# yukara-ikemiya/friendly-stable-audio-tools

Hardware: AMD Instinct MI355X
Metric: audio-seconds/sec @44.1kHz stereo, 100-step DPM++, SA-Open-1.0 shape (higher is better)
Workload: dtype fp16; 1 GPU; Stable-Audio-Open-1.0 DiT shape (24 layers, D=1536, S=1025, CFG 7 -> 2 sequences/prompt) + Oobleck decode, 1 prompt(s)/GPU x 47.55 s, 100 DPM-Solver++(3M) SDE steps; prompts_per_gpu=1, codec_dtype=fp16, sampler_steps=100, layernorm=fused, cross_attention=fused, sample_size=2097152, parallelism=dp1 (rank-strided prompts, one all-gather)

## Files before the change

### friendly-stable-audio-tools_amd/csrc/gemm_bf16.hip

```cpp
#include <stdlib.h>

#include <type_traits>

#include "attn_core.h"
#include <algorithm>

#include "sat_common.h"

namespace {

template <int EPI, int MI, int NI, bool LNC = false, bool QKN = false>
__device__ __forceinline__ void gemm_epilogue(const GemmArgs& g, f32x16 (&acc)[MI][NI], const int mw, const int nw, const int half,
                                              const int l31, const float2* ln = nullptr, const float* lc1 = nullptr,
                                              const float* lc2 = nullptr) {
    const int M = g.M, N = g.N;
    (void)N;

    if constexpr (EPI == EPI_F32) {
        float* __restrict__ C = g.C;
        const int ldc = g.ldc;
        float bia[NI];
#pragma unroll
        for (int j = 0; j < NI; ++j) bia[j] = g.bias ? g.bias[nw + j * 32 + l31] : 0.f;
        const bool accum = g.accumulate != 0;
// ... 344 lines not shown
            const int m = mw + i * 32 + l31;
            const int mc = m < M ? m : M - 1;
            const int b = mc / S;
            const int s = mc - b * S;
            const int ob = (kind & 4) ? ((b * S) & 3) : 0;
            if constexpr (LNC) {
                const float2 st = ln[i * 32 + l31];
#pragma unroll
                for (int j = 0; j < 2; ++j)
#pragma unroll
                    for (int q = 0; q < 4; ++q) {
                        const f32x4 c1 = *reinterpret_cast<const f32x4*>(lc1 + j * 32 + q * 8 + 4 * half);
                        const f32x4 c2 = *reinterpret_cast<const f32x4*>(lc2 + j * 32 + q * 8 + 4 * half);
#pragma unroll
                        for (int e = 0; e < 4; ++e) acc[i][j][4 * q + e] = st.y * (acc[i][j][4 * q + e] - st.x * c1[e]) + c2[e];
                    }
            }
            if constexpr (QKN) {
                if (kind & 16) {
                    float ss = 0.f;
#pragma unroll
                    for (int j = 0; j < 2; ++j)
#pragma unroll
                        for (int r = 0; r < 16; ++r) ss += acc[i][j][r] * acc[i][j][r];
                    unsigned a = __float_as_uint(ss), b = a;
                    half_swap(a, b);
                    const float inv = rsqrtf(fmaxf(__uint_as_float(a) + __uint_as_float(b), 1e-24f));
#pragma unroll
                    for (int j = 0; j < 2; ++j)
#pragma unroll
                        for (int r = 0; r < 16; ++r) acc[i][j][r] *= inv;
                }
            }
            if (kind & 2) {
                if constexpr (!ROPE_PRE) {
                    rcs[i][0] = *reinterpret_cast<const f32x4*>(he.rope_cos + (size_t)s * 16 + 4 * half);
                    rcs[i][1] = *reinterpret_cast<const f32x4*>(he.rope_cos + (size_t)s * 16 + 8 + 4 * half);
                    rsn[i][0] = *reinterpret_cast<const f32x4*>(he.rope_sin + (size_t)s * 16 + 4 * half);
                    rsn[i][1] = *reinterpret_cast<const f32x4*>(he.rope_sin + (size_t)s * 16 + 8 + 4 * half);
                }
                const f32x4 cs0 = rcs[i][0], cs1 = rcs[i][1], sn0 = rsn[i][0], sn1 = rsn[i][1];
#pragma unroll
                for (int r = 0; r < 8; ++r) {
                    const float cs = (r < 4) ? cs0[r & 3] : cs1[r & 3];
                    const float sn = (r < 4) ? sn0[r & 3] : sn1[r & 3];
                    const float x1 = acc[i][0][r], x2 = acc[i][0][r + 8];
                    acc[i][0][r] = x1 * cs - x2 * sn;
                    acc[i][0][r + 8] = x2 * cs + x1 * sn;
                }
            }
            if (kind & 8) {
#pragma unroll
                for (int j = 0; j < 2; ++j)
#pragma unroll
                    for (int r = 0; r < 16; ++r) acc[i][j][r] *= he.qscale;
            }
            op_t* row = dst + ((size_t)(b * he.heads + head) * Spad + s + ob) * 64 + 8 * half;
#pragma unroll
            for (int j = 0; j < 2; ++j) {
                unsigned pk[8];
#pragma unroll
                for (int q = 0; q < 4; ++q) {
                    pk[2 * q] = pack_op2(acc[i][j][4 * q], acc[i][j][4 * q + 1]);
                    pk[2 * q + 1] = pack_op2(acc[i][j][4 * q + 2], acc[i][j][4 * q + 3]);
                }
                half_swap(pk[0], pk[2]);
                half_swap(pk[1], pk[3]);
                half_swap(pk[4], pk[6]);
                half_swap(pk[5], pk[7]);
                if (qfrag) {
#pragma unroll
                    for (int e = 0; e < 8; ++e) qfrag[j][e] = pk[e];
                    continue;
                }
                if (m < M) {
                    *reinterpret_cast<u32x4*>(row + j * 32) = u32x4{pk[0], pk[1], pk[2], pk[3]};
                    *reinterpret_cast<u32x4*>(row + j * 32 + 16) = u32x4{pk[4], pk[5], pk[6], pk[7]};
                }
            }
        }
    }
}

template <int MI>
__device__ __forceinline__ void stage_rows32(float* ep, const f32x16 (&acc)[MI][2], const int i, const int lane) {
    const int half = lane >> 5, l31 = lane & 31;
#pragma unroll
    for (int j = 0; j < 2; ++j)
#pragma unroll
        for (int r = 0; r < 16; ++r) ep[((r & 3) + 8 * (r >> 2) + 4 * half) * 64 + j * 32 + l31] = acc[i][j][r];
}
template <int MB>
__device__ __forceinline__ void stage_rows32(float* ep, const f32x4 (&acc)[MB][4], const int i, const int lane) {
    const int l15 = lane & 15, q = lane >> 4;
#pragma unroll
    for (int rb = 0; rb < 2; ++rb)
#pragma unroll
        for (int cb = 0; cb < 4; ++cb)
#pragma unroll
            for (int r = 0; r < 4; ++r) ep[(rb * 16 + 4 * q + r) * 64 + cb * 16 + l15] = acc[2 * i + rb][cb][r];
}

template <int MI, bool PRE = false, typename Acc>
__device__ __forceinline__ void gemm_epilogue_f32_staged(const GemmArgs& g, Acc& acc, float* ep, const int mw, const int nw,
                                                         const int lane, const f32x4* pre = nullptr) {
    const int M = g.M;
    const int prow = lane >> 4;
    const int c4 = (lane & 15) * 4;
    const bool accum = g.accumulate != 0;
    const f32x4 bia = g.bias ? *reinterpret_cast<const f32x4*>(g.bias + nw + c4) : f32x4{0.f, 0.f, 0.f, 0.f};
#pragma unroll
    for (int i = 0; i < MI; ++i) {
        stage_rows32(ep, acc, i, lane);
#pragma unroll
        for (int grp = 0; grp < 2; ++grp) {
            f32x4 old[4];
#pragma unroll
            for (int p4 = 0; p4 < 4; ++p4) {
                const int m = mw + i * 32 + (grp * 4 + p4) * 4 + prow;
                if constexpr (PRE) old[p4] = pre[grp * 4 + p4];
                else old[p4] = (accum && m < M) ? *reinterpret_cast<const f32x4*>(g.C + (size_t)m * g.ldc + nw + c4) : f32x4{0.f, 0.f, 0.f, 0.f};
            }
#pragma unroll
            for (int p4 = 0; p4 < 4; ++p4) {
                const int row = (grp * 4 + p4) * 4 + prow;
                const int m = mw + i * 32 + row;
                f32x4 v = *reinterpret_cast<const f32x4*>(ep + row * 64 + c4) + bia;
                if (m < M && g.gate) v *= *reinterpret_cast<const f32x4*>(g.gate + (size_t)(m / g.gate_rows) * g.gate_ld + nw + c4);
                v += old[p4];
                if (m < M) *reinterpret_cast<f32x4*>(g.C + (size_t)m * g.ldc + nw + c4) = v;
                if (g.xb) {
                    opx4 xr;
                    float sum = 0.f, sq = 0.f;
#pragma unroll
                    for (int e = 0; e < 4; ++e) {
                        xr[e] = f32_to_op(v[e]);
                        const float f = op_to_f32(xr[e]);
                        sum += f;
                        sq += f * f;
                    }
                    sum = row16_sum(sum);
                    sq = row16_sum(sq);
                    if (m < M) {
                        *reinterpret_cast<opx4*>(g.xb + (size_t)m * g.N + nw + c4) = xr;
                        if ((lane & 15) == 0)
                            *reinterpret_cast<float2*>(g.ln_part_out + ((size_t)m * (g.N >> 6) + (nw >> 6)) * 2) = make_float2(sum, sq);
                    }
                }
            }
        }
    }
}

template <int BM, int BN, int WM, int WN, int EPIX>
__global__ __launch_bounds__(WM * WN * 64) void gemm_kernel(GemmArgs g) {
    sat_f16_saturate();
    constexpr int EPI = EPIX == EPI_HEADS_QKN ? EPI_HEADS : EPIX == EPI_ACT16 ? EPI_SWIGLU : EPIX;
    constexpr bool QKN = EPIX == EPI_HEADS_QKN || EPIX == EPI_ACT16;
    constexpr int NT = WM * WN * 64;
    constexpr int TM = BM / WM;
    constexpr int TN = BN / WN;
    static_assert(TN == 64, "wave tile is TM x 64");
    constexpr int MI = TM / 32;
    constexpr int NI = 2;
    constexpr int A_CH = BM * 8 / NT;
    constexpr int B_CH = BN * 8 / NT;
// ... 164 lines not shown
        int q = i * NT + tid;
        int row = q >> 3, pos = q & 7;
        int c = pos ^ ((row >> 1) & 7);
        b_ptr[i] = g.W + (size_t)(n0 + row) * K + c * 8;
    }

    f32x16 acc[MI][NI];
#pragma unroll
    for (int i = 0; i < MI; ++i)
#pragma unroll
        for (int j = 0; j < NI; ++j)
#pragma unroll
            for (int r = 0; r < 16; ++r) acc[i][j][r] = 0.f;

    auto stage_in = [&](int kt, int stage) {
        char* sa = smem + stage * STAGE_BYTES;
        char* sb = sa + BM * 128;
#pragma unroll
        for (int i = 0; i < A_CH; ++i)
            __builtin_amdgcn_global_load_lds((const __attribute__((address_space(1))) void*)(a_ptr[i] + kt * 64),
                                             (__attribute__((address_space(3))) void*)(sa + (i * NT + wave * 64) * 16), 16, 0, 0);
#pragma unroll
        for (int i = 0; i < B_CH; ++i)
            __builtin_amdgcn_global_load_lds((const __attribute__((address_space(1))) void*)(b_ptr[i] + kt * 64),
                                             (__attribute__((address_space(3))) void*)(sb + (i * NT + wave * 64) * 16), 16, 0, 0);
    };
    auto compute = [&](int stage) {
        const char* sa = smem + stage * STAGE_BYTES;
        const char* sb = sa + BM * 128;
#pragma unroll
        for (int ks = 0; ks < 4; ++ks) {
            opx8 af[MI], bfr[NI];
#pragma unroll
            for (int i = 0; i < MI; ++i)
                af[i] = *reinterpret_cast<const opx8*>(sa + lds_tile_off(wm * TM + i * 32 + l31, ks * 2 + half));
#pragma unroll
            for (int j = 0; j < NI; ++j)
                bfr[j] = *reinterpret_cast<const opx8*>(sb + lds_tile_off(wn * TN + j * 32 + l31, ks * 2 + half));
#pragma unroll
            for (int i = 0; i < MI; ++i)
#pragma unroll
                for (int j = 0; j < NI; ++j)
                    acc[i][j] = mfma_32x32x16(af[i], bfr[j], acc[i][j]);
        }
    };

    const int nk = K / 64;
    stage_in(0, 0);
    __syncthreads();
    for (int kt = 0; kt < nk - 1; ++kt) {
        stage_in(kt + 1, (kt + 1) & 1);
        compute(kt & 1);
        __syncthreads();
    }
    compute((nk - 1) & 1);

    gemm_epilogue<EPI, MI, NI, false, QKN>(g, acc, m0 + wm * TM, n0 + wn * TN, half, l31);
}

#ifdef SAT_RING_MFMA_32X32
constexpr bool SAT_RING_MFMA_16 = false;
#else
constexpr bool SAT_RING_MFMA_16 = true;
#endif

template <int BK>
__device__ __forceinline__ int lds_off_bk(int row, int chunk) {
    if constexpr (BK == 128) return row * 256 + ((chunk ^ (row & 15)) << 4);
    else if constexpr (BK == 64) return row * 128 + ((chunk ^ ((row >> 1) & 7)) << 4);
    else return row * 64 + ((chunk ^ ((row >> 2) & 3)) << 4);
}

template <int BM, int BN, int BK, int WM, int WN, int NS, int EPIX, int FP8 = 0, int KG = 1, bool DIL = false>
__global__ __launch_bounds__(KG * WM * WN * 64) void gemm_pipe_kernel(GemmArgs g) {
    sat_f16_saturate();
    constexpr int EPI = EPIX == EPI_HEADS_QKN ? EPI_HEADS : EPIX == EPI_ACT16 ? EPI_SWIGLU : EPIX;
    constexpr bool QKN = EPIX == EPI_HEADS_QKN || EPIX == EPI_ACT16;
    static_assert(!QKN || FP8 == 0, "qk_norm / plain activation: 16-bit operands only");
    static_assert(KG == 1 || (KG == 2 && EPI == EPI_F32 && FP8 == 0 && BK == 64 && BM / WM == 64 && BN / WN == 64),
                  "K-groups: fp32 output, 64 x 64 wave tiles, 128-byte rows");
    constexpr int NT = KG * WM * WN * 64;
    constexpr int TM = BM / WM;
    constexpr int TN = BN / WN;
    constexpr bool S16 = SAT_RING_MFMA_16 && EPI == EPI_F32 && FP8 == 0 && NT == 512;
    static_assert(!S16 || BK == 64, "16 x 16 x 32 fragments: two 32-k steps per 128-byte row");
    static_assert(TN == 64, "wave tile is TM x 64");
    constexpr int MI = TM / 32;
    constexpr int NI = TN / 32;
    constexpr int CPR = BK / 8;
    constexpr int NW = KG * WM * WN;
    constexpr int WL_A = BM * CPR / 64;
    constexpr int WLG = (BM + BN) * CPR / 64;
    constexpr int WL = KG * WLG;
    constexpr int LPT = (WL + NW - 1) / NW;
    constexpr int N_FULL = WL - (LPT - 1) * NW;
    constexpr bool UNIFORM = (WL % NW) == 0;
    constexpr int ROWB = BK * 2;
    constexpr bool MXA = FP8 == 3;
    constexpr int SCALE_WAVES = MXA ? BM / 64 : 0;
    constexpr int GROUP_BYTES = (BM + BN) * ROWB + (MXA ? BM * 4 : 0);
    constexpr int STAGE_BYTES = KG * GROUP_BYTES;
    constexpr int D = NS - 1;
    constexpr bool DIL_ON = (DIL || KG == 2) && FP8 == 0;
    constexpr int NDIL = !DIL_ON ? 0 : UNIFORM ? LPT : LPT - 1;
    constexpr int DIL_STEPS = KG == 2 ? (S16 ? 1 : BK / 32) : BK / 16 - 1;
    static_assert(!S16 || KG == 2 || !DIL_ON, "16 x 16 x 32, one K-group: the LDS-DMA pieces are issued in front of compute()");
    constexpr int DIL_PER = (NDIL + DIL_STEPS - 1) / (DIL_STEPS > 0 ? DIL_STEPS : 1);
    static_assert(!MXA || D == 1 || UNIFORM, "MXFP8: counted waits are built for uniform tiles or 2-stage rings");
    static_assert((BM * CPR) % 64 == 0 && (BN * CPR) % 64 == 0 && (D - 1) * LPT < 64, "bad pipeline geometry");
    static_assert(!FP8 || BK == 64, "fp8: 128-byte rows only");

    extern __shared__ __attribute__((aligned(16))) char smem[];

    const int tid = threadIdx.x;
    const int lane = tid & 63;
    const int wave = __builtin_amdgcn_readfirstlane(tid >> 6);
    const int grp = KG == 2 ? wave / (WM * WN) : 0;
    const int wv = KG == 2 ? wave % (WM * WN) : wave;
    const int wm = wv / WN;
    const int wn = wv % WN;
    const int half = lane >> 5;
    const int l31 = lane & 31;

    const int M = g.M, N = g.N, K = g.K;
    const int tiles_m = (M + BM - 1) / BM;
    const int tiles_n = N / BN;
    const int bid = xcd_remap(blockIdx.x, gridDim.x);
    int tm, tn;
    if (tiles_m <= tiles_n) {
        tn = bid / tiles_m;
        tm = bid - tn * tiles_m;
    } else {
        tm = bid / tiles_n;
        tn = bid - tm * tiles_n;
    }
    const int m0 = tm * BM;
    const int n0 = tn * BN;
    const bool wave_rows_valid = (m0 + wm * TM) < M;
    constexpr bool XA_OK = EPI == EPI_HEADS && MI == 1 && NI == 2 && NW == 4 && BN == 64 && BK == 64 && NS == 3 && FP8 == 0;
    constexpr int XA_OFF = (NS * STAGE_BYTES + (BM + BN) * 8 + 1023) & ~1023;
    [[maybe_unused]] bool xa_on = false;
    [[maybe_unused]] auto xa_stage = [&](int b) {
        const HeadsEpi& he = g.heads;
        const int kvh = (n0 >> 6) / (he.heads / he.xa_kvh);
        const op_t* kbase = he.xa_k + (size_t)(b * he.xa_kvh + kvh) * he.xa_sk_pad * 64;
        const op_t* vbase = he.xa_vt + (size_t)(b * he.xa_kvh + kvh) * 64 * he.xa_sk_pad;
        const int n_t = (((b * he.xa_sk) & 3) + he.xa_sk + 63) >> 6;
        for (int t = 0; t < n_t; ++t)
#pragma unroll
            for (int i = 0; i < 2; ++i) {
                const int p = wave + 4 * i;
                const int row = p * 8 + (lane >> 3);
                const int c = (lane & 7) ^ ((row >> 1) & 7);
                char* dst = smem + XA_OFF + t * 16384 + p * 1024;
                __builtin_amdgcn_global_load_lds((const __attribute__((address_space(1))) void*)(kbase + (size_t)(t * 64 + row) * 64 + c * 8),
                                                 (__attribute__((address_space(3))) void*)dst, 16, 0, 0);
                __builtin_amdgcn_global_load_lds((const __attribute__((address_space(1))) void*)(vbase + (size_t)row * he.xa_sk_pad + t * 64 + c * 8),
                                                 (__attribute__((address_space(3))) void*)(dst + 8192), 16, 0, 0);
            }
    };
    if constexpr (XA_OK) {
        xa_on = g.heads.xa_k != nullptr;
        if (xa_on) xa_stage(m0 / g.heads.S);
    }
    constexpr bool PRE_RESID = EPI == EPI_F32 && (MI == 1 || KG == 2) && NI == 2 && NT <= 512;
    const int epi_m = m0 + wm * TM + (KG == 2 ? grp * 32 : 0);
    const bool epi_rows_valid = KG == 2 ? epi_m < M : wave_rows_valid;
// ... 110 lines not shown
                if constexpr (MXA) {
                    static_assert(!TRc, "MXFP8 A operand: block scales were probed on the A side only (tools/mx_probe.cpp)");
                    if (ks == 0) return __builtin_amdgcn_mfma_scale_f32_32x32x64_f8f6f4(af_, bf_, c_, 0, 0, 0, sdw[i], 0, 0x7F7F7F7F);
                    return __builtin_amdgcn_mfma_scale_f32_32x32x64_f8f6f4(af_, bf_, c_, 0, 0, 2, sdw[i], 0, 0x7F7F7F7F);
                } else if constexpr (TRc) {
                    return __builtin_amdgcn_mfma_scale_f32_32x32x64_f8f6f4(bf_, af_, c_, 0, 0, 0, 0x7F7F7F7F, 0, 0x7F7F7F7F);
                } else {
                    return __builtin_amdgcn_mfma_scale_f32_32x32x64_f8f6f4(af_, bf_, c_, 0, 0, 0, 0x7F7F7F7F, 0, 0x7F7F7F7F);
                }
            };
            if constexpr (!DBUF) {
#pragma unroll
                for (int ks = 0; ks < KS2; ++ks) {
                    frag(ks, 0);
#pragma unroll
                    for (int i = 0; i < MI; ++i)
#pragma unroll
                        for (int j = 0; j < NI; ++j)
                            acc[i][j] = mx(af[0][i], bfr[0][j], acc[i][j], ks, i);
                }
                return;
            }
            frag(0, 0);
            __builtin_amdgcn_sched_group_barrier(0x100, 2 * (MI + NI), 0);
#pragma unroll
            for (int ks = 0; ks < KS2; ++ks) {
                if (ks + 1 < KS2) frag(ks + 1, (ks + 1) & 1);
#pragma unroll
                for (int i = 0; i < MI; ++i)
#pragma unroll
                    for (int j = 0; j < NI; ++j)
                        acc[i][j] = mx(af[ks & 1][i], bfr[ks & 1][j], acc[i][j], ks, i);
                if (ks + 1 < KS2) {
                    constexpr int NR = 2 * (MI + NI), NM = MI * NI;
#pragma unroll
                    for (int r = 0; r < NM; ++r) {
                        __builtin_amdgcn_sched_group_barrier(0x8, 1, 0);
                        __builtin_amdgcn_sched_group_barrier(0x100, NR / NM, 0);
                    }
                    if (NR % NM) __builtin_amdgcn_sched_group_barrier(0x100, NR % NM, 0);
                } else {
                    __builtin_amdgcn_sched_group_barrier(0x8, MI * NI, 0);
                }
            }
            return;
        }
        if constexpr (FP8 == 1) {
            i64x2 af[2][MI], bfr[2][NI];
            auto frag = [&](int ks, int buf) {
#pragma unroll
                for (int i = 0; i < MI; ++i)
                    af[buf][i] = *reinterpret_cast<const i64x2*>(sa + lds_off_bk<BK>(wm * TM + i * 32 + l31, ks * 2 + half));
#pragma unroll
                for (int j = 0; j < NI; ++j)
                    bfr[buf][j] = *reinterpret_cast<const i64x2*>(sb + lds_off_bk<BK>(wn * TN + j * 32 + l31, ks * 2 + half));
            };
            frag(0, 0);
            __builtin_amdgcn_sched_group_barrier(0x100, MI + NI, 0);
#pragma unroll
            for (int ks = 0; ks < KS; ++ks) {
                if (ks + 1 < KS) frag(ks + 1, (ks + 1) & 1);
#pragma unroll
                for (int h2 = 0; h2 < 2; ++h2)
#pragma unroll
                    for (int i = 0; i < MI; ++i)
#pragma unroll
                        for (int j = 0; j < NI; ++j)
                            acc[i][j] = TRc ? __builtin_amdgcn_mfma_f32_32x32x16_fp8_fp8(bfr[ks & 1][j][h2], af[ks & 1][i][h2], acc[i][j], 0, 0, 0)
                                            : __builtin_amdgcn_mfma_f32_32x32x16_fp8_fp8(af[ks & 1][i][h2], bfr[ks & 1][j][h2], acc[i][j], 0, 0, 0);
                if (ks + 1 < KS) {
#pragma unroll
                    for (int r = 0; r < MI + NI; ++r) {
                        __builtin_amdgcn_sched_group_barrier(0x8, 1, 0);
                        __builtin_amdgcn_sched_group_barrier(0x100, 1, 0);
                    }
                    __builtin_amdgcn_sched_group_barrier(0x8, 2 * MI * NI - (MI + NI), 0);
                } else {
                    __builtin_amdgcn_sched_group_barrier(0x8, 2 * MI * NI, 0);
                }
            }
            return;
        }
        if constexpr (S16) {
            static_assert(!TRc, "16 x 16 x 32: fp32 output, un-swapped");
            constexpr int KS2 = BK / 32, NR = MB + 4, NM = MB * 4;
            const int l15 = lane & 15, q = lane >> 4;
            opx8 af[2][MB], bfr[2][4];
            auto frag = [&](int ks, int buf) {
#pragma unroll
                for (int i = 0; i < MB; ++i)
                    af[buf][i] = *reinterpret_cast<const opx8*>(sa + lds_off_bk<BK>(wm * TM + i * 16 + l15, ks * 4 + q));
#pragma unroll
                for (int j = 0; j < 4; ++j)
                    bfr[buf][j] = *reinterpret_cast<const opx8*>(sb + lds_off_bk<BK>(wn * TN + j * 16 + l15, ks * 4 + q));
            };
            frag(0, 0);
            __builtin_amdgcn_sched_group_barrier(0x100, NR, 0);
#pragma unroll
            for (int ks = 0; ks < KS2; ++ks) {
                if (ks + 1 < KS2) frag(ks + 1, (ks + 1) & 1);
                if constexpr (KG == 2) {
                    if (ks < DIL_STEPS && kt_issue >= 0) {
                        char* sdst = smem + st_issue * STAGE_BYTES;
#pragma unroll
                        for (int i = ks * DIL_PER; i < (ks + 1) * DIL_PER && i < NDIL; ++i)
                            __builtin_amdgcn_global_load_lds((const __attribute__((address_space(1))) void*)(ld_ptr[i] + kt_issue * (BK * KG)),
                                                             (__attribute__((address_space(3))) void*)(sdst + (grp * WLG + i * (WM * WN) + wv) * 1024), 16, 0, 0);
                    }
                }
#pragma unroll
                for (int i = 0; i < MB; ++i)
#pragma unroll
                    for (int j = 0; j < 4; ++j) acc16[i][j] = mfma_16x16x32(af[ks & 1][i], bfr[ks & 1][j], acc16[i][j]);
                if constexpr (KG == 2) {
                    if (ks + 1 < KS2) {
                        __builtin_amdgcn_sched_group_barrier(0x8, 1, 0);
                        __builtin_amdgcn_sched_group_barrier(0x100, NR / 2, 0);
                        __builtin_amdgcn_sched_group_barrier(0x8, 1, 0);
                        __builtin_amdgcn_sched_group_barrier(0x100, NR - NR / 2, 0);
                        if (DIL_PER == 8 && NM == 16) {
                            __builtin_amdgcn_sched_group_barrier(0x8, 1, 0);
#pragma unroll
                            for (int r = 0; r < 4; ++r) {
                                __builtin_amdgcn_sched_group_barrier(0x8, 1, 0);
                                __builtin_amdgcn_sched_group_barrier(0x20, 2, 0);
                                __builtin_amdgcn_sched_group_barrier(0x8, 2, 0);
                            }
                            __builtin_amdgcn_sched_group_barrier(0x8, 1, 0);
                        } else {
                            __builtin_amdgcn_sched_group_barrier(0x8, NM - 2, 0);
                        }
                    } else {
                        __builtin_amdgcn_sched_group_barrier(0x8, NM, 0);
                    }
                    if (ks == KS2 / 2 - 1) {
                        __builtin_amdgcn_sched_barrier(0);
                        __builtin_amdgcn_s_barrier();
                        __builtin_amdgcn_sched_barrier(0);
                    }
                } else if (ks + 1 < KS2) {
#pragma unroll
                    for (int r = 0; r < (NR < NM ? NR : NM); ++r) {
                        __builtin_amdgcn_sched_group_barrier(0x8, 1, 0);
                        __builtin_amdgcn_sched_group_barrier(0x100, 1, 0);
                    }
                    if (NM > NR) __builtin_amdgcn_sched_group_barrier(0x8, NM - NR, 0);
                    if (NR > NM) __builtin_amdgcn_sched_group_barrier(0x100, NR - NM, 0);
                } else {
                    __builtin_amdgcn_sched_group_barrier(0x8, NM, 0);
                }
            }
            return;
        }
        opx8 af[2][MI], bfr[2][NI];
        auto frag = [&](int ks, int buf) {
#pragma unroll
            for (int i = 0; i < MI; ++i)
                af[buf][i] = *reinterpret_cast<const opx8*>(sa + lds_off_bk<BK>(wm * TM + i * 32 + l31, ks * 2 + half));
#pragma unroll
            for (int j = 0; j < NI; ++j)
                bfr[buf][j] = *reinterpret_cast<const opx8*>(sb + lds_off_bk<BK>(wn * TN + j * 32 + l31, ks * 2 + half));
        };
        frag(0, 0);
        __builtin_amdgcn_sched_group_barrier(0x100, MI + NI, 0);
#pragma unroll
        for (int ks = 0; ks < KS; ++ks) {
            if (ks + 1 < KS) frag(ks + 1, (ks + 1) & 1);
            if constexpr (DIL_ON) {
                if (ks < DIL_STEPS && kt_issue >= 0) {
                    char* sdst = smem + st_issue * STAGE_BYTES;
#pragma unroll
                    for (int i = ks * DIL_PER; i < (ks + 1) * DIL_PER && i < NDIL; ++i)
                        __builtin_amdgcn_global_load_lds((const __attribute__((address_space(1))) void*)(ld_ptr[i] + kt_issue * (BK * KG)),
                                                         (__attribute__((address_space(3))) void*)(sdst + (KG == 2 ? grp * WLG + i * (WM * WN) + wv : i * NW + wave) * 1024), 16, 0, 0);
                }
            }
#pragma unroll
            for (int i = 0; i < MI; ++i)
#pragma unroll
                for (int j = 0; j < NI; ++j)
                    acc[i][j] = TRc ? mfma_32x32x16(bfr[ks & 1][j], af[ks & 1][i], acc[i][j])
                                    : mfma_32x32x16(af[ks & 1][i], bfr[ks & 1][j], acc[i][j]);
            if (ks + 1 < KS) {
                constexpr int NR = MI + NI, NM = MI * NI;
                if constexpr (KG == 2) {
                    __builtin_amdgcn_sched_group_barrier(0x8, 1, 0);
                    __builtin_amdgcn_sched_group_barrier(0x100, NR, 0);
                    if (ks < KS / 2 && DIL_PER == 4) {
                        __builtin_amdgcn_sched_group_barrier(0x8, 1, 0);
                        __builtin_amdgcn_sched_group_barrier(0x20, 2, 0);
                        __builtin_amdgcn_sched_group_barrier(0x8, 1, 0);
                        __builtin_amdgcn_sched_group_barrier(0x20, 2, 0);
                        __builtin_amdgcn_sched_group_barrier(0x8, 1, 0);
                    } else {
                        __builtin_amdgcn_sched_group_barrier(0x8, NM - 1, 0);
                    }
// ... 187 lines not shown
                    const float sa_r = g.a_scale[row];
#pragma unroll
                    for (int j = 0; j < NI; ++j)
#pragma unroll
                        for (int q = 0; q < 4; ++q) {
                            const f32x4 sw = *reinterpret_cast<const f32x4*>(g.w_scale + n0 + wn * TN + j * 32 + q * 8 + 4 * half);
#pragma unroll
                            for (int e = 0; e < 4; ++e) acc[i][j][4 * q + e] *= sa_r * sw[e];
                        }
                }
            } else {
                float sw[NI];
#pragma unroll
                for (int j = 0; j < NI; ++j) sw[j] = g.w_scale[n0 + wn * TN + j * 32 + l31];
#pragma unroll
                for (int i = 0; i < MI; ++i)
#pragma unroll
                    for (int r = 0; r < 16; ++r) {
                        int row = m0 + wm * TM + i * 32 + (r & 3) + 8 * (r >> 2) + 4 * half;
                        row = row < M ? row : M - 1;
                        const float sa_r = MXA ? 1.0f : g.a_scale[row];
#pragma unroll
                        for (int j = 0; j < NI; ++j) acc[i][j][r] *= sa_r * sw[j];
                    }
            }
        }
    }
    if constexpr (KG == 2) {
        __builtin_amdgcn_s_barrier();
        if constexpr (S16) {
            f32x4* mine = reinterpret_cast<f32x4*>(smem) + wave * 512;
#pragma unroll
            for (int rb = 0; rb < 2; ++rb)
#pragma unroll
                for (int cb = 0; cb < 4; ++cb) {
                    f32x4 v;
#pragma unroll
                    for (int e = 0; e < 4; ++e) v[e] = grp ? acc16[rb][cb][e] : acc16[2 + rb][cb][e];
                    mine[(rb * 4 + cb) * 64 + lane] = v;
                }
            __syncthreads();
            const f32x4* theirs = reinterpret_cast<const f32x4*>(smem) + (wave ^ (WM * WN)) * 512;
            f32x4 fin[2][4];
#pragma unroll
            for (int rb = 0; rb < 2; ++rb)
#pragma unroll
                for (int cb = 0; cb < 4; ++cb) {
                    const f32x4 t = theirs[(rb * 4 + cb) * 64 + lane];
#pragma unroll
                    for (int e = 0; e < 4; ++e) fin[rb][cb][e] = (grp ? acc16[2 + rb][cb][e] : acc16[rb][cb][e]) + t[e];
                }
            if (epi_rows_valid)
                gemm_epilogue_f32_staged<1, true>(g, fin, reinterpret_cast<float*>(smem + NW * 8192) + wave * 2048, epi_m, n0 + wn * TN, lane, resid);
            return;
        }
        float* mine = reinterpret_cast<float*>(smem) + wave * 2048;
#pragma unroll
        for (int j = 0; j < 2; ++j)
#pragma unroll
            for (int r = 0; r < 16; ++r) mine[(j * 16 + r) * 64 + lane] = grp ? acc[0][j][r] : acc[1][j][r];
        __syncthreads();
        const float* theirs = reinterpret_cast<const float*>(smem) + (wave ^ (WM * WN)) * 2048;
        f32x16 fin[1][2];
#pragma unroll
        for (int j = 0; j < 2; ++j)
#pragma unroll
            for (int r = 0; r < 16; ++r) fin[0][j][r] = (grp ? acc[1][j][r] : acc[0][j][r]) + theirs[(j * 16 + r) * 64 + lane];
        static_assert(KG == 1 || NS * STAGE_BYTES >= 2 * NW * 8192, "exchange + staging areas");
        if (epi_rows_valid)
            gemm_epilogue_f32_staged<1, true>(g, fin, reinterpret_cast<float*>(smem + NW * 8192) + wave * 2048, epi_m, n0 + wn * TN, lane, resid);
        return;
    }
    if constexpr (EPI == EPI_F32) {
        __builtin_amdgcn_s_barrier();
        if (wave_rows_valid) {
            if constexpr (S16 && PRE_RESID)
                gemm_epilogue_f32_staged<MI, true>(g, acc16, reinterpret_cast<float*>(smem) + wave * 2048, m0 + wm * TM, n0 + wn * TN, lane, resid);
            else if constexpr (S16)
                gemm_epilogue_f32_staged<MI>(g, acc16, reinterpret_cast<float*>(smem) + wave * 2048, m0 + wm * TM, n0 + wn * TN, lane);
            else if constexpr (PRE_RESID)
                gemm_epilogue_f32_staged<MI, true>(g, acc, reinterpret_cast<float*>(smem) + wave * 2048, m0 + wm * TM, n0 + wn * TN, lane, resid);
            else
                gemm_epilogue_f32_staged<MI>(g, acc, reinterpret_cast<float*>(smem) + wave * 2048, m0 + wm * TM, n0 + wn * TN, lane);
        }
    } else if (wave_rows_valid) {
        if (tr) gemm_epilogue_t<EPI, MI, NI, LN_CONS, (NT < 1024), QKN>(g, acc, m0 + wm * TM, n0 + wn * TN, half, l31, lnst + wm * TM, lnc + wn * TN, lnc + BN + wn * TN);
        else gemm_epilogue<EPI, MI, NI, LN_CONS, QKN>(g, acc, m0 + wm * TM, n0 + wn * TN, half, l31, lnst + wm * TM, lnc + wn * TN, lnc + BN + wn * TN);
    }
}

template <int BM, int BN, int BK, int WM, int WN, int NS, int EPIX, int FP8 = 0, int KG = 1, bool DIL = false>
int launch_pipe(const GemmArgs& a, hipStream_t stream) {
    constexpr int EPI = EPIX == EPI_HEADS_QKN ? EPI_HEADS : EPIX == EPI_ACT16 ? EPI_SWIGLU : EPIX;
    constexpr int NT = KG * WM * WN * 64;
    constexpr bool LN_CONS = (EPI == EPI_SWIGLU || EPI == EPI_HEADS) && FP8 == 0;
    constexpr int LDS = NS * KG * ((BM + BN) * BK * 2 + (FP8 == 3 ? BM * 4 : 0)) + (LN_CONS ? (BM + BN) * 8 : 0);
    static_assert(LDS <= 160 * 1024, "LDS ring exceeds 160 KiB");
    SAT_CHECK_ARG(LN_CONS || !a.ln_part, SAT_E_UNSUPPORTED, "gemm: LayerNorm fold needs bf16 operands and a SwiGLU / heads epilogue");
    SAT_CHECK_ARG((!a.xb && !a.ln_part_out) || (EPI == EPI_F32 && BN / WN == 64 && FP8 == 0 && a.xb && a.ln_part_out), SAT_E_UNSUPPORTED,
                  "gemm: the bf16 image / row statistics come from the bf16 fp32-output tiles with 64-column wave tiles");
    static_assert(EPI != EPI_F32 || BN / WN != 64 || LDS >= WM * WN * 8192, "the staged fp32 epilogue needs 8 KiB of LDS per wave");
    auto kern = gemm_pipe_kernel<BM, BN, BK, WM, WN, NS, EPIX, FP8, KG, DIL>;
    constexpr bool XA_OK = EPI == EPI_HEADS && BM == 128 && BN == 64 && BK == 64 && WM == 4 && WN == 1 && NS == 3 && FP8 == 0;
    constexpr int XA_LDS = XA_OK ? ((NS * (BM + BN) * BK * 2 + (BM + BN) * 8 + 1023) & ~1023) + 3 * 16384 : LDS;
    static_assert(XA_LDS <= 160 * 1024, "fused cross-attention: K / V^T tiles do not fit behind the ring");
    bool xa = false;
    if constexpr (EPI == EPI_HEADS) {
        xa = a.heads.xa_k != nullptr;
        if (xa) {
            const HeadsEpi& he = a.heads;
            SAT_CHECK_ARG(XA_OK, SAT_E_UNSUPPORTED, "gemm: the fused cross-attention epilogue lives in the 128 x 64 tile (variant 16)");
            SAT_CHECK_ARG(he.parts == 1 && (he.kind[0] & ~16) == 8 && he.qscale == SAT_ATTN_QSCALE && he.xa_vt && he.xa_out && he.xa_kvh > 0 &&
                              he.heads % he.xa_kvh == 0 && he.xa_sk > 0 && he.xa_sk + 3 <= 192 && he.xa_sk_pad >= he.xa_sk + 3 && he.xa_sk_pad % 64 == 0,
                          SAT_E_UNSUPPORTED, "gemm: fused cross-attention needs one pre-scaled row-major part and at most 189 keys (got %d)", he.xa_sk);
        }
    }
    SAT_TRY(sat_ensure_dynamic_lds(reinterpret_cast<const void*>(kern), XA_LDS));
    GemmArgs b = a;
    if (FP8) {
        SAT_CHECK_ARG(a.K % 128 == 0 && a.w_scale && (FP8 == 3 ? (const void*)a.a_bscale : (const void*)a.a_scale), SAT_E_UNSUPPORTED,
                      "gemm(fp8): K=%d must be a multiple of 128 and both scale vectors given", a.K);
        b.K = a.K / 2;
    }
    SAT_CHECK_ARG(b.N % BN == 0, SAT_E_UNSUPPORTED, "gemm: N=%d not a multiple of the %d-column tile", b.N, BN);
    SAT_CHECK_ARG(b.K % (BK * KG) == 0 && b.K / (BK * KG) >= NS, SAT_E_UNSUPPORTED, "gemm: K=%d too small for the %d-stage pipeline", a.K, NS);
    int tiles = cdiv(b.M, BM) * (b.N / BN);
    hipLaunchKernelGGL(kern, dim3(tiles), dim3(NT), xa ? XA_LDS : LDS, stream, b);
    SAT_LAUNCH_CHECK();
    return 0;
}

template <int BM, int BN, int WM, int WN, int EPI, bool GLDS = false>
int launch_cfg(const GemmArgs& a, hipStream_t stream) {
    constexpr int NT = WM * WN * 64;
    constexpr int LDS = 2 * (BM + BN) * 128;
    SAT_CHECK_ARG(!a.ln_part && !a.xb && !a.ln_part_out, SAT_E_UNSUPPORTED, "gemm: LayerNorm fold is built into the pipelined tiles only (K >= 192)");
    auto kern = GLDS ? gemm_glds_kernel<BM, BN, WM, WN, EPI> : gemm_kernel<BM, BN, WM, WN, EPI>;
    SAT_TRY(sat_ensure_dynamic_lds(reinterpret_cast<const void*>(kern), LDS));
    SAT_CHECK_ARG(a.N % BN == 0, SAT_E_UNSUPPORTED, "gemm: N=%d not a multiple of the %d-column tile", a.N, BN);
    int tiles = cdiv(a.M, BM) * (a.N / BN);
    hipLaunchKernelGGL(kern, dim3(tiles), dim3(NT), LDS, stream, a);
    SAT_LAUNCH_CHECK();
    return 0;
}

template <int ID, int EPI, int F8>
int launch_tile(const GemmArgs& a, hipStream_t stream) {
    constexpr SatTile t = sat_tile_geom(ID);
    static_assert(!t.f32_only || EPI == EPI_F32, "tile built for the fp32-output epilogue only");
    if constexpr (t.family == SAT_GEMM_PIPE) return launch_pipe<t.bm, t.bn, t.bk, t.wm, t.wn, t.ns, EPI, F8, t.kg, t.dil && F8 == 0>(a, stream);
    else return launch_cfg<t.bm, t.bn, t.wm, t.wn, EPI, t.family == SAT_GEMM_DMA2>(a, stream);
}

template <int EPI, int F8>
int launch_epi(int tile, const GemmArgs& a, hipStream_t stream) {
#define SAT_TILE_CASE(id) \
    case id: return launch_tile<id, EPI, F8>(a, stream);
    switch (tile) {
        SAT_TILE_CASE(SAT_TILE_128)
        SAT_TILE_CASE(SAT_TILE_128x64)
        SAT_TILE_CASE(SAT_TILE_256)
        SAT_TILE_CASE(SAT_TILE_256x192)
    }
    if constexpr (F8 == 0) {
        switch (tile) {
            SAT_TILE_CASE(SAT_TILE_REF_128)
// ... 98 lines not shown
```

Baseline: 77.68 audio-seconds/sec.

## Use 16x16x32 MFMA fragments for 768-thread heads-epilogue GEMM tiles

Extends the 16x16x32 MFMA ring path, previously limited to fp32-output 512-thread tiles, to the QKV heads epilogue with 768-thread tiles (no qk-norm). It adds dedicated epilogues for the 16x16 accumulator layout: a row-major path that applies the LayerNorm fold, RoPE and q-scale and uses permlane16 swaps to assemble contiguous stores, and a transposed V path. The intent is better MFMA throughput or register pressure for the QKV projection. In exchange it adds new layout-specific store code, including exact RoPE rounding handling, that must match the existing 32x32 epilogue bit for bit.

```diff
diff --git a/friendly-stable-audio-tools_amd/csrc/gemm_bf16.hip b/friendly-stable-audio-tools_amd/csrc/gemm_bf16.hip
--- a/friendly-stable-audio-tools_amd/csrc/gemm_bf16.hip
+++ b/friendly-stable-audio-tools_amd/csrc/gemm_bf16.hip
@@ -450,6 +450,174 @@
     }
 }
 
+__device__ __forceinline__ void row16_swap(unsigned& a, unsigned& b) {
+    u32x2 r = __builtin_amdgcn_permlane16_swap(a, b, false, false);
+    a = r[0];
+    b = r[1];
+}
+
+template <int MB, bool LNC>
+__device__ __forceinline__ void gemm_heads16_t(const GemmArgs& g, f32x4 (&acc)[MB][4], const int mw, const int nw, const int lane,
+                                               const float2* ln, const float* lc1, const float* lc2) {
+    const int M = g.M;
+    const int l15 = lane & 15, qt = lane >> 4;
+    const HeadsEpi& he = g.heads;
+    const int hp = he.heads * 64;
+    const int part = nw / hp;
+    const int head = (nw - part * hp) >> 6;
+    const int kind = he.kind[part];
+    op_t* __restrict__ dst = he.out[part];
+    const int S = he.S, Spad = he.Spad;
+    [[maybe_unused]] f32x4 rcs[MB], rsn[MB];
+    if (kind & 2) {
+#pragma unroll
+        for (int i = 0; i < MB; ++i) {
+            const int m = mw + i * 16 + l15;
+            const int s = (m < M ? m : M - 1) % S;
+            rcs[i] = *reinterpret_cast<const f32x4*>(he.rope_cos + (size_t)s * 16 + 4 * qt);
+            rsn[i] = *reinterpret_cast<const f32x4*>(he.rope_sin + (size_t)s * 16 + 4 * qt);
+        }
+    }
+    [[maybe_unused]] f32x4 c1[4], c2[4];
+    if constexpr (LNC) {
+#pragma unroll
+        for (int j = 0; j < 4; ++j) {
+            c1[j] = *reinterpret_cast<const f32x4*>(lc1 + j * 16 + 4 * qt);
+            c2[j] = *reinterpret_cast<const f32x4*>(lc2 + j * 16 + 4 * qt);
+        }
+    }
+    const int crun = 16 * (qt & 1) + 8 * (qt >> 1);
+#pragma unroll
+    for (int i = 0; i < MB; ++i) {
+        const int m = mw + i * 16 + l15;
+        const int mc = m < M ? m : M - 1;
+        const int b = mc / S;
+        const int s = mc - b * S;
+        const int ob = (kind & 4) ? ((b * S) & 3) : 0;
+        if constexpr (LNC) {
+            const float2 st = ln[i * 16 + l15];
+#pragma unroll
+            for (int j = 0; j < 4; ++j)
+#pragma unroll
+                for (int e = 0; e < 4; ++e) acc[i][j][e] = st.y * (acc[i][j][e] - st.x * c1[j][e]) + c2[j][e];
+        }
+        if (kind & 2) {
+#pragma clang fp contract(off)
+#pragma unroll
+            for (int e = 0; e < 4; ++e) {
+                const float cs = rcs[i][e], sn = rsn[i][e];
+                const float x1 = acc[i][0][e], x2 = acc[i][1][e];
+                const float t = x2 * cs;
+                float hi = __builtin_fmaf(x1, sn, t);
+                if (e >= 2) {
+                    const float u = x1 * sn;
+                    hi = qt >= 2 ? t + u : hi;
+                }
+                acc[i][0][e] = __builtin_fmaf(x1, cs, -(x2 * sn));
+                acc[i][1][e] = hi;
+            }
+        }
+        if (kind & 8) {
+#pragma unroll
+            for (int j = 0; j < 4; ++j)
+#pragma unroll
+                for (int e = 0; e < 4; ++e) acc[i][j][e] *= he.qscale;
+        }
+        op_t* row = dst + ((size_t)(b * he.heads + head) * Spad + s + ob) * 64 + crun;
+#pragma unroll
+        for (int jp = 0; jp < 2; ++jp) {
+            unsigned a0 = pack_op2(acc[i][2 * jp][0], acc[i][2 * jp][1]), a1 = pack_op2(acc[i][2 * jp][2], acc[i][2 * jp][3]);
+            unsigned b0 = pack_op2(acc[i][2 * jp + 1][0], acc[i][2 * jp + 1][1]), b1 = pack_op2(acc[i][2 * jp + 1][2], acc[i][2 * jp + 1][3]);
+            row16_swap(a0, b0);
+            row16_swap(a1, b1);
+            if (m < M) *reinterpret_cast<u32x4*>(row + jp * 32) = u32x4{a0, a1, b0, b1};
+        }
+    }
+}
+
+template <int MB, bool LNC>
+__device__ __forceinline__ void gemm_heads16_vt(const GemmArgs& g, f32x4 (&acc)[MB][4], const int mw, const int nw, const int lane,
+                                                const float2* ln, const float* lc1, const float* lc2) {
+    const int M = g.M;
+    const int l15 = lane & 15, qt = lane >> 4;
+    const HeadsEpi& he = g.heads;
+    const int hp = he.heads * 64;
+    const int part = nw / hp;
+    const int head = (nw - part * hp) >> 6;
+    const int kind = he.kind[part];
+    op_t* __restrict__ dst = he.out[part];
+    const int S = he.S, Spad = he.Spad;
+    const bool shift = (kind & 4) != 0;
+    [[maybe_unused]] float c1[4], c2[4];
+    if constexpr (LNC) {
+#pragma unroll
+        for (int j = 0; j < 4; ++j) {
+            c1[j] = lc1[j * 16 + l15];
+            c2[j] = lc2[j * 16 + l15];
+        }
+    }
+#pragma unroll
+    for (int i = 0; i < MB; ++i) {
+        const int mb = mw + i * 16 + 4 * qt;
+        float v[4][4];
+        int bb[4], ss[4];
+        f32x4 st01 = {0.f, 1.f, 0.f, 1.f}, st23 = {0.f, 1.f, 0.f, 1.f};
+        if constexpr (LNC) {
+            const f32x4* sp = reinterpret_cast<const f32x4*>(ln + i * 16 + 4 * qt);
+            st01 = sp[0];
+            st23 = sp[1];
+        }
+#pragma unroll
+        for (int e = 0; e < 4; ++e) {
+            int mm = mb + e;
+            mm = mm < M ? mm : M - 1;
+            bb[e] = mm / S;
+            ss[e] = mm - bb[e] * S;
+#pragma unroll
+            for (int j = 0; j < 4; ++j) {
+                v[j][e] = acc[i][j][e];
+                if constexpr (LNC) {
+                    const float mean = e < 2 ? st01[2 * e] : st23[2 * e - 4];
+                    const float rstd = e < 2 ? st01[2 * e + 1] : st23[2 * e - 3];
+                    v[j][e] = rstd * (v[j][e] - mean * c1[j]) + c2[j];
+                }
+            }
+            if (kind & 2) {
+                const float cs = he.rope_cos[ss[e] * 16 + l15], sn = he.rope_sin[ss[e] * 16 + l15];
+                const float x1 = v[0][e], x2 = v[1][e];
+                v[0][e] = x1 * cs - x2 * sn;
+                v[1][e] = x2 * cs + x1 * sn;
+            }
+        }
+        if (mb + 3 < M && bb[0] == bb[3]) {
+            const int ob = shift ? ((bb[0] * S) & 3) : 0;
+            const size_t hbase = ((size_t)(bb[0] * he.heads + head) * 64) * Spad;
+            const size_t base = hbase + vt_pos(ss[0] + ob);
+#pragma unroll
+            for (int j = 0; j < 4; ++j) {
+                opx4 p;
+#pragma unroll
+                for (int e = 0; e < 4; ++e) p[e] = f32_to_op(v[j][e]);
+                if (shift) {
+                    *reinterpret_cast<opx4*>(dst + base + (size_t)(j * 16 + l15) * Spad) = p;
+                } else {
+#pragma unroll
+                    for (int e = 0; e < 4; ++e) dst[hbase + vt_pos(ss[0] + e) + (size_t)(j * 16 + l15) * Spad] = p[e];
+                }
+            }
+        } else {
+#pragma unroll
+            for (int e = 0; e < 4; ++e)
+                if (mb + e < M) {
+                    const int ob = shift ? ((bb[e] * S) & 3) : 0;
+                    const size_t base = ((size_t)(bb[e] * he.heads + head) * 64) * Spad + vt_pos(ss[e] + ob);
+#pragma unroll
+                    for (int j = 0; j < 4; ++j) dst[base + (size_t)(j * 16 + l15) * Spad] = f32_to_op(v[j][e]);
+                }
+        }
+    }
+}
+
 template <int MI>
 __device__ __forceinline__ void stage_rows32(float* ep, const f32x16 (&acc)[MI][2], const int i, const int lane) {
     const int half = lane >> 5, l31 = lane & 31;
@@ -780,7 +948,7 @@
     constexpr int NT = KG * WM * WN * 64;
     constexpr int TM = BM / WM;
     constexpr int TN = BN / WN;
-    constexpr bool S16 = SAT_RING_MFMA_16 && EPI == EPI_F32 && FP8 == 0 && NT == 512;
+    constexpr bool S16 = SAT_RING_MFMA_16 && FP8 == 0 && ((EPI == EPI_F32 && NT == 512) || (EPI == EPI_HEADS && !QKN && NT == 768));
     static_assert(!S16 || BK == 64, "16 x 16 x 32 fragments: two 32-k steps per 128-byte row");
     static_assert(TN == 64, "wave tile is TM x 64");
     constexpr int MI = TM / 32;
@@ -1057,7 +1225,7 @@
             return;
         }
         if constexpr (S16) {
-            static_assert(!TRc, "16 x 16 x 32: fp32 output, un-swapped");
+            static_assert(!TRc || EPI == EPI_HEADS, "16 x 16 x 32: fp32 output is un-swapped");
             constexpr int KS2 = BK / 32, NR = MB + 4, NM = MB * 4;
             const int l15 = lane & 15, q = lane >> 4;
             opx8 af[2][MB], bfr[2][4];
@@ -1086,7 +1254,9 @@
 #pragma unroll
                 for (int i = 0; i < MB; ++i)
 #pragma unroll
-                    for (int j = 0; j < 4; ++j) acc16[i][j] = mfma_16x16x32(af[ks & 1][i], bfr[ks & 1][j], acc16[i][j]);
+                    for (int j = 0; j < 4; ++j)
+                        acc16[i][j] = TRc ? mfma_16x16x32(bfr[ks & 1][j], af[ks & 1][i], acc16[i][j])
+                                          : mfma_16x16x32(af[ks & 1][i], bfr[ks & 1][j], acc16[i][j]);
                 if constexpr (KG == 2) {
                     if (ks + 1 < KS2) {
                         __builtin_amdgcn_sched_group_barrier(0x8, 1, 0);
@@ -1440,6 +1610,11 @@
                 gemm_epilogue_f32_staged<MI, true>(g, acc, reinterpret_cast<float*>(smem) + wave * 2048, m0 + wm * TM, n0 + wn * TN, lane, resid);
             else
                 gemm_epilogue_f32_staged<MI>(g, acc, reinterpret_cast<float*>(smem) + wave * 2048, m0 + wm * TM, n0 + wn * TN, lane);
+        }
+    } else if constexpr (S16) {
+        if (wave_rows_valid) {
+            if (tr) gemm_heads16_t<MB, LN_CONS>(g, acc16, m0 + wm * TM, n0 + wn * TN, lane, lnst + wm * TM, lnc + wn * TN, lnc + BN + wn * TN);
+            else gemm_heads16_vt<MB, LN_CONS>(g, acc16, m0 + wm * TM, n0 + wn * TN, lane, lnst + wm * TM, lnc + wn * TN, lnc + BN + wn * TN);
         }
     } else if (wave_rows_valid) {
         if (tr) gemm_epilogue_t<EPI, MI, NI, LN_CONS, (NT < 1024), QKN>(g, acc, m0 + wm * TM, n0 + wn * TN, half, l31, lnst + wm * TM, lnc + wn * TN, lnc + BN + wn * TN);
```

New measurement: 78.65 audio-seconds/sec (median of 6 runs). 1.2% higher.
